# dev-wei/recman

Measured on AMD Instinct MI355X. Metric: examples/sec fwd+bwd, Criteo-shape batch 65536; % HBM and MFMA roofline, higher is better.
Workload: dtype f32; 1 GPU; deepfm (BASELINE configs[1]); batch_per_gpu=65536, batch_all_gpus=65536, sparse_fields=26, rows_per_field=1000001, dense_fields=13, emb_dim=16, indices=uniform, table_row_loads=cached (rm_deepfm_step), row_gradient_stores=cached (as in fit(): the optimizer step gathers them next), optimizer_step=excluded, matrix_arithmetic=f32 MFMA (v_mfma_f32_16x16x4_f32), fp32 accumulate, hipgraph=True, table=single GPU

## Files before the change

### recman_amd/csrc/step.hip

```cpp
#include "mlp_internal.h"
#include "rm_common.h"

namespace {

typedef float f32x4 __attribute__((ext_vector_type(4)));
typedef unsigned u32x4 __attribute__((ext_vector_type(4)));
typedef __amdgpu_buffer_rsrc_t rsrc_t;

constexpr int kWorkers = 7;
constexpr int kSlots = 4;
constexpr int kMaxF = 26;
constexpr int kRing = 3;
constexpr int kSlotB = 1024;
constexpr int kXBufB = kMaxF * kSlotB;
constexpr int kPartH = 0, kPartS = 2048, kPartQ = 3072, kPartSd = 3328, kPartB = 3584;
constexpr int kLDT = 36;
constexpr int kPubDh = 0, kPubDT = 2048, kPubGS = kPubDT + 16 * kLDT * 4, kPubG = kPubGS + 1024, kPubB = kPubG + 256;
constexpr int oX = 0;
constexpr int oDense = oX + kRing * kXBufB;
constexpr int oJunk = oDense + 4 * kSlotB;
constexpr int oZero = oJunk + kSlotB;
constexpr int oPart = oZero + kSlotB;
constexpr int oPub = oPart + 2 * kWorkers * kPartB;
constexpr int kRowB = 28 * 64;
constexpr int oRow = oPub + 2 * kPubB;
constexpr int oHT = oRow + 2 * kRowB;
constexpr int oD1T = oHT + 16 * 32 * 4;
constexpr int oY = oD1T + 16 * 32 * 4;
constexpr int oW1 = oY + 4 * 16 * 4;
constexpr int oPar = oW1 + 32 * 32 * 4;
constexpr int kParB0 = 0, kParB1 = 128, kParWo = 256, kParWd = 384, kParFo = 448;
constexpr int kLdsBytes = oPar + 448 + 28 * 4;
static_assert(kLdsBytes <= 160 * 1024, "LDS map exceeds a CU");

#ifndef RM_STEP_ABL
#define RM_STEP_ABL 0
#endif
#ifdef RM_STEP_STAMP
__device__ unsigned long long rm_step_stamp_buf[256 * 8 * 8];
#define ST_NOW() __builtin_amdgcn_s_memtime()
#define ST_DECL unsigned long long st_acc[8] = {0, 0, 0, 0, 0, 0, 0, 0}, st_t = ST_NOW(), st_t0 = st_t
#define ST_ADD(i) { const unsigned long long st_n = ST_NOW(); st_acc[i] += st_n - st_t; st_t = st_n; }
#define ST_FLUSH(wv) if (lane == 0 && blockIdx.x < 256) { st_acc[7] = ST_NOW() - st_t0; for (int i_ = 0; i_ < 8; ++i_) rm_step_stamp_buf[(blockIdx.x * 8 + (wv)) * 8 + i_] = st_acc[i_]; }
#else
#define ST_DECL
#define ST_ADD(i)
#define ST_FLUSH(wv)
#endif

struct StepArgs {
  const int64_t *idx, *field_off;
  const char *table;
  unsigned row_bytes;
  const float *dense;
  const int64_t *y;
  const float *y_f;
  const float *W0, *b0, *W1, *b1, *w_out, *w0_out, *lin_wd, *lin_w0;
  int F, Dn, H0, H1, act, task, Kp;
  float grad_scale;
  int64_t B;
  float *d_rows, *logit, *pred, *dlogit, *dW0_part, *sg_part, *loss_part;
  int packed, out_row_bytes, out_rows;
  const float *lin_mask;
};

__device__ __forceinline__ float act_slope(int act) {
  return act == RM_ACT_RELU ? 0.f : (act == RM_ACT_LEAKY_RELU ? 0.2f : 1.f);
}
__device__ __forceinline__ float actf(float v, float slope) { return v > 0.f ? v : slope * v; }
__device__ __forceinline__ float actg(float o, float slope) { return o > 0.f ? 1.f : slope; }

__device__ __forceinline__ int slot_field(int w, int j) {
  return j < 3 ? 7 * j + w : (w < 3 ? 21 + w : (w > 3 ? 20 + w : -1));
}

__device__ __forceinline__ f32x4 mfma16(float a, float b, f32x4 c) {
  return __builtin_amdgcn_mfma_f32_16x16x4f32(a, b, c, 0, 0, 0);
}
__device__ __forceinline__ f32x4 mfma16w(float a, float b, f32x4 c) {
  if (RM_STEP_ABL & 16) { c.x += a * b; return c; }
  return __builtin_amdgcn_mfma_f32_16x16x4f32(a, b, c, 0, 0, 0);
}

__device__ __forceinline__ constexpr int swz(int r) { return ((r >> 3) & 1) * 3; }

template <bool NT>
__device__ __forceinline__ void dma16(const char *src, char *lds_dst) {
  __builtin_amdgcn_global_load_lds((const __attribute__((address_space(1))) void *)src,
                                   (__attribute__((address_space(3))) void *)lds_dst, 16, 0, NT ? 2 : 0);
}

template <class T>
__device__ __forceinline__ void entry_load(T &dst, const void *src) {
  static_assert(sizeof(T) == 4, "one dword");
  asm volatile("global_load_dword %0, %1, off" : "=v"(dst) : "v"(src) : "memory");
}
template <int YOUNGER>
__device__ __forceinline__ void entry_wait(float &v) {
  asm volatile("s_waitcnt vmcnt(%1)" : "+v"(v) : "n"(YOUNGER) : "memory");
}

typedef float f32x2 __attribute__((ext_vector_type(2)));
template <int OFF, class T>
__device__ __forceinline__ void lds_load(T &dst, unsigned addr) {
  static_assert(sizeof(T) == 4 || sizeof(T) == 16, "b32 or b128");
  if (sizeof(T) == 4) asm volatile("ds_read_b32 %0, %1 offset:%2" : "=v"(dst) : "v"(addr), "n"(OFF) : "memory");
  else asm volatile("ds_read_b128 %0, %1 offset:%2" : "=v"(dst) : "v"(addr), "n"(OFF) : "memory");
}
__device__ __forceinline__ void lds_load_pair(f32x2 &dst, unsigned addr) {
  asm volatile("ds_read2st64_b32 %0, %1 offset1:1" : "=v"(dst) : "v"(addr) : "memory");
}
struct SlotRegs {
  f32x2 col[2];
  f32x4 e4;
};
#define RM_SLOT_REGS(r) "+v"((r).col[0]), "+v"((r).col[1]), "+v"((r).e4)
template <bool PACKED>
__device__ __forceinline__ void slot_wait0(f32x4 (&dhB)[2], float (&dT)[2][4], f32x4 &gS, float &g, unsigned (&rid)[4],
                                           unsigned (&rp0)[4], SlotRegs &r) {
  if (PACKED)
    asm volatile("s_waitcnt lgkmcnt(9)"
                 : "+v"(dhB[0]), "+v"(dhB[1]), "+v"(dT[0][0]), "+v"(dT[0][1]), "+v"(dT[0][2]), "+v"(dT[0][3]),
                   "+v"(dT[1][0]), "+v"(dT[1][1]), "+v"(dT[1][2]), "+v"(dT[1][3]), "+v"(gS), "+v"(g), "+v"(rid[0]),
                   "+v"(rid[1]), "+v"(rid[2]), "+v"(rid[3]), "+v"(rp0[0]), "+v"(rp0[1]), "+v"(rp0[2]), "+v"(rp0[3]),
                   RM_SLOT_REGS(r)::"memory");
  else
    asm volatile("s_waitcnt lgkmcnt(9)"
                 : "+v"(dhB[0]), "+v"(dhB[1]), "+v"(dT[0][0]), "+v"(dT[0][1]), "+v"(dT[0][2]), "+v"(dT[0][3]),
                   "+v"(dT[1][0]), "+v"(dT[1][1]), "+v"(dT[1][2]), "+v"(dT[1][3]), "+v"(gS), "+v"(g), "+v"(rid[0]),
                   "+v"(rid[1]), "+v"(rid[2]), "+v"(rid[3]), RM_SLOT_REGS(r)::"memory");
}
__device__ __forceinline__ void slot_wait(int j, SlotRegs &r) {
  if (j == 1) asm volatile("s_waitcnt lgkmcnt(6)" : RM_SLOT_REGS(r)::"memory");
  else if (j == 2) asm volatile("s_waitcnt lgkmcnt(3)" : RM_SLOT_REGS(r)::"memory");
  else asm volatile("s_waitcnt lgkmcnt(0)" : RM_SLOT_REGS(r)::"memory");
}
static_assert(kSlots == 4, "slot_wait's counts");

__device__ __forceinline__ void wait_vm(int younger) {
#define RM_WV(N) case N: asm volatile("s_waitcnt vmcnt(" #N ")" ::: "memory"); break;
  switch (younger) {
    RM_WV(24) RM_WV(23) RM_WV(22) RM_WV(21) RM_WV(20) RM_WV(19) RM_WV(18) RM_WV(17) RM_WV(16) RM_WV(15) RM_WV(14) RM_WV(13) RM_WV(12) RM_WV(11) RM_WV(10) RM_WV(9) RM_WV(8) RM_WV(7) RM_WV(6)
    RM_WV(5) RM_WV(4) RM_WV(3) RM_WV(2) RM_WV(1)
    default: asm volatile("s_waitcnt vmcnt(0)" ::: "memory"); break;
  }
#undef RM_WV
}

__device__ __forceinline__ void tile_barrier() {
  asm volatile("s_waitcnt lgkmcnt(0)" ::: "memory");
  __builtin_amdgcn_s_barrier();
  asm volatile("" ::: "memory");
}

__device__ __forceinline__ float sum_q(float v) {
  {
    float a = v, c = v;
    asm("s_nop 1\n\tv_permlane16_swap_b32 %0, %1" : "+v"(a), "+v"(c));
    v = a + c;
  }
  {
    float a = v, c = v;
    asm("s_nop 1\n\tv_permlane32_swap_b32 %0, %1" : "+v"(a), "+v"(c));
    v = a + c;
  }
  return v;
}
__device__ __forceinline__ float sum_n(float v) {
#pragma unroll
  for (int o = 1; o < 16; o <<= 1) v += __shfl_xor(v, o, 64);
  return v;
}

template <bool NT, bool NT_OUT, bool PACKED>
__device__ __forceinline__ void step_worker(const StepArgs &a, char *smem, const int w, const int lane, const int T) {
  const int n = lane & 15, q = lane >> 4;
  const int F = a.F, H0 = a.H0, K = 16 * F + a.Dn;
  int fld[kSlots];
  bool sv[kSlots], sx[kSlots];
  float w0f[kSlots][2][4];
  float w0x[kSlots][2][4];
  f32x4 dw[kSlots][2];
#pragma unroll
  for (int j = 0; j < kSlots; ++j) {
    const int f = slot_field(w, j);
    sv[j] = f >= 0 && (f < F || (f == F && a.Dn > 0));
    sx[j] = f >= 0 && f < F;
    fld[j] = sv[j] ? f : 0;
    const int kb = 16 * fld[j];
#pragma unroll
    for (int uh = 0; uh < 2; ++uh) {
#pragma unroll
      for (int e = 0; e < 4; ++e) {
        const int kf = kb + 4 * q + e, uf = 16 * uh + n;
        const bool okf = sv[j] && kf < K && uf < H0;
        const float vf = a.W0[okf ? (int64_t)kf * H0 + uf : 0];
        w0f[j][uh][e] = okf ? vf : 0.f;
        const int kx = kb + n, ux = 16 * uh + 4 * q + e;
        const bool okx = sx[j] && kx < K && ux < H0;
        const float vx = a.W0[okx ? (int64_t)kx * H0 + ux : 0];
        w0x[j][uh][e] = okx ? vx : 0.f;
      }
      dw[j][uh] = f32x4{0.f, 0.f, 0.f, 0.f};
    }
  }
  const int64_t tstride = gridDim.x;
  const int lo_slice = n * 64 + 16 * (q ^ swz(n));
  int lo_col[2];
#pragma unroll
  for (int h = 0; h < 2; ++h) lo_col[h] = (8 * h + q) * 64 + 16 * ((n >> 2) ^ swz(8 * h + q)) + 4 * (n & 3);
  static_assert(swz(0) == swz(4) && swz(3) == swz(7) && swz(8) == swz(12) && swz(11) == swz(15), "a pair of column reads shares its swizzle");
  const unsigned lds0 = (unsigned)(uintptr_t)(__attribute__((address_space(3))) char *)smem;
  const int lo_row = n * F * 64 + 16 * q;
  auto slot_base = [&](int j, int tile) {
    const int ring = oX + ((tile + 6) % 3) * kXBufB + fld[j] * kSlotB, dn = oDense + (tile & 3) * kSlotB;
    return __builtin_amdgcn_readfirstlane(sx[j] ? ring : (sv[j] ? dn : oZero));
  };
  *reinterpret_cast<f32x4 *>(smem + oZero + lane * 16) = f32x4{0.f, 0.f, 0.f, 0.f};
  const int piece = 16 * ((lane & 3) ^ swz(lane >> 2));
  const int side_off = 64 + 4 * (lane & 1);
  float sdv[kSlots];
#pragma unroll
  for (int j = 0; j < kSlots; ++j) sdv[j] = 0.f;
  unsigned rp[4][kSlots];
  float lmask[kSlots];
#pragma unroll
  for (int j = 0; j < kSlots; ++j) {
    rp[0][j] = rp[1][j] = rp[2][j] = rp[3][j] = 0;
    lmask[j] = (PACKED && a.lin_mask != nullptr && sx[j]) ? a.lin_mask[fld[j]] : 1.f;
  }
  constexpr int kSP = PACKED ? 2 : 1;
  constexpr int kYoungerE = 7 + 4 * kSP, kYounger = 8 + 6 * kSP;
  static_assert(kYounger <= 24, "wait_vm's range");
  asm volatile("" ::"s"(a.row_bytes) : "memory");
  ST_DECL;
  ST_ADD(0);

  for (int s = -2; s <= T + 1; ++s) {
    const bool hasB = s - 2 >= 0 && s - 2 < T;
    const bool hasD = s + 1 >= 0 && s + 1 < T;
    float side_sum = 0.f;
    {
      const int tb = s - 2, td = s + 1;
      char *xd = smem + oX + ((td + 3) % 3) * kXBufB;
      f32x4 dhB[2], gS;
      float dT[2][4], g;
      SlotRegs sr[kSlots];
      unsigned rid[kSlots];
      {
        const unsigned pub = lds0 + oPub + (tb & 1) * kPubB;
        lds_load<kPubDh>(dhB[0], pub + lane * 16);
        lds_load<kPubDh + 1024>(dhB[1], pub + lane * 16);
        const unsigned pt = pub + (q * kLDT + n) * 4;
#pragma unroll
        for (int uh = 0; uh < 2; ++uh) {
          lds_load<kPubDT + (0 * 4 * kLDT) * 4>(dT[uh][0], pt + 64 * uh);
          lds_load<kPubDT + (1 * 4 * kLDT) * 4>(dT[uh][1], pt + 64 * uh);
          lds_load<kPubDT + (2 * 4 * kLDT) * 4>(dT[uh][2], pt + 64 * uh);
          lds_load<kPubDT + (3 * 4 * kLDT) * 4>(dT[uh][3], pt + 64 * uh);
        }
        lds_load<kPubGS>(gS, pub + lane * 16);
        lds_load<kPubG>(g, pub + lane * 4);
      }
      if (PACKED) {
#pragma unroll
        for (int j = 0; j < kSlots; ++j) {
          rp[3][j] = rp[2][j];
          rp[2][j] = rp[1][j];
          rp[1][j] = rp[0][j];
        }
      }
// ... 84 lines not shown
      }
    }
    ST_ADD(6);
    if (s >= 0 && s < T) {
      wait_vm(kYounger);
      ST_ADD(3);
      f32x4 acc0 = f32x4{0.f, 0.f, 0.f, 0.f}, acc1 = acc0, S = acc0, Q = acc0;
      f32x4 x4[kSlots];
#pragma unroll
      for (int j = 0; j < kSlots; ++j) {
        x4[j] = *reinterpret_cast<const f32x4 *>(smem + slot_base(j, s) + lo_slice);
      }
#pragma unroll
      for (int j = 0; j < kSlots; ++j) {
#pragma unroll
        for (int ks = 0; ks < 4; ++ks) {
          acc0 = mfma16w(w0f[j][0][ks], x4[j][ks], acc0);
          acc1 = mfma16w(w0f[j][1][ks], x4[j][ks], acc1);
        }
        const float m = sx[j] ? 1.f : 0.f;
        S += m * x4[j];
        Q += m * (x4[j] * x4[j]);
      }
      char *part = smem + oPart + ((s & 1) * kWorkers + w) * kPartB;
      *reinterpret_cast<f32x4 *>(part + kPartH + lane * 16) = acc0;
      *reinterpret_cast<f32x4 *>(part + kPartH + (64 + lane) * 16) = acc1;
      *reinterpret_cast<f32x4 *>(part + kPartS + lane * 16) = S;
      *reinterpret_cast<float *>(part + kPartQ + lane * 4) = (Q.x + Q.y) + (Q.z + Q.w);
      *reinterpret_cast<float *>(part + kPartSd + lane * 4) = side_sum;
    }
    ST_ADD(4);
    tile_barrier();
    ST_ADD(5);
  }
  asm volatile("s_waitcnt vmcnt(0)" ::: "memory");
#pragma unroll
  for (int j = 0; j < kSlots; ++j)
    if (sv[j]) {
#pragma unroll
      for (int uh = 0; uh < 2; ++uh)
#pragma unroll
        for (int i = 0; i < 4; ++i)
          a.dW0_part[((int64_t)blockIdx.x * a.Kp + 16 * fld[j] + 4 * q + i) * 32 + 16 * uh + n] = dw[j][uh][i];
    }
  ST_ADD(0);
  ST_FLUSH(w);
}

__device__ __forceinline__ void step_head(const StepArgs &a, char *smem, const int lane, const int T) {
  const int n = lane & 15, q = lane >> 4;
  const int F = a.F, Dn = a.Dn, H0 = a.H0, H1 = a.H1;
  const float act = act_slope(a.act);
  const int64_t B = a.B, tstride = gridDim.x;
  {
    float *w1s = reinterpret_cast<float *>(smem + oW1);
#pragma unroll
    for (int i = 0; i < 16; ++i) {
      const int e = lane + 64 * i, u = e >> 5, v = e & 31;
      const bool ok = u < H0 && v < H1;
      const float f = a.W1[ok ? u * H1 + v : 0];
      w1s[u * 32 + 4 * ((v >> 2) ^ (u & 7)) + (v & 3)] = ok ? f : 0.f;
    }
    float *par = reinterpret_cast<float *>(smem + oPar);
    if (lane < 32) {
      const float f0 = a.b0[lane < H0 ? lane : 0], f1 = a.b1[lane < H1 ? lane : 0], f2 = a.w_out[lane < H1 ? lane : 0];
      par[kParB0 / 4 + lane] = lane < H0 ? f0 : 0.f;
      par[kParB1 / 4 + lane] = lane < H1 ? f1 : 0.f;
      par[kParWo / 4 + lane] = lane < H1 ? f2 : 0.f;
      const float f3 = a.lin_wd[lane < Dn ? lane : 0];
      if (lane < 16) par[kParWd / 4 + lane] = lane < Dn ? f3 : 0.f;
      if (lane < 28) reinterpret_cast<unsigned *>(par)[kParFo / 4 + lane] = (unsigned)a.field_off[lane < F ? lane : F - 1];
    }
  }
  const float *w1s = reinterpret_cast<const float *>(smem + oW1);
  const char *par = smem + oPar;
  const float w0o = a.w0_out[0], lw0 = a.lin_w0[0];

  f32x4 dW1[2][2];
  float db0[2][4], db1[2][4], dwo[2][4], dxd[4], sg = 0.f, loss_acc = 0.f;
#pragma unroll
  for (int x = 0; x < 2; ++x)
#pragma unroll
    for (int i = 0; i < 4; ++i) {
      dW1[x][0][i] = dW1[x][1][i] = 0.f;
      db0[x][i] = db1[x][i] = dwo[x][i] = 0.f;
    }
#pragma unroll
  for (int i = 0; i < 4; ++i) dxd[i] = 0.f;

  auto ex_of = [&](int t) {
    const int64_t b = ((int64_t)blockIdx.x + t * tstride) * 16 + n;
    return b < B ? b : B - 1;
  };
  unsigned idr[7];
  float dnr[4];
  unsigned yr = 0;
#pragma unroll
  for (int j = 0; j < 7; ++j) idr[j] = 0;
#pragma unroll
  for (int i = 0; i < 4; ++i) dnr[i] = 0.f;
  auto load_ids = [&](int t) {
    const unsigned *p = reinterpret_cast<const unsigned *>(a.idx + ex_of(t) * F);
#pragma unroll
    for (int j = 0; j < 7; ++j) entry_load(idr[j], p + 2 * (q + 4 * j < F ? q + 4 * j : F - 1));
  };
  asm volatile("" ::"v"(w0o), "v"(lw0) : "memory");
  load_ids(0);
  ST_DECL;
  ST_ADD(0);

  for (int s = -2; s <= T + 1; ++s) {
    const bool epi = s - 1 >= 0 && s - 1 < T;
    float o_z = 0.f, o_p = 0.f, o_g = 0.f;
    if (epi) {
      const int t = s - 1;
      const int64_t bex = ((int64_t)blockIdx.x + t * tstride) * 16 + n;
      const bool valid = bex < B;
      f32x4 pre[2], S = f32x4{0.f, 0.f, 0.f, 0.f};
      pre[0] = pre[1] = S;
      float ss = 0.f, y1 = 0.f, ls = 0.f;
#pragma unroll
      for (int w = 0; w < kWorkers; ++w) {
        const char *part = smem + oPart + ((t & 1) * kWorkers + w) * kPartB;
        pre[0] += *reinterpret_cast<const f32x4 *>(part + kPartH + lane * 16);
        pre[1] += *reinterpret_cast<const f32x4 *>(part + kPartH + (64 + lane) * 16);
        S += *reinterpret_cast<const f32x4 *>(part + kPartS + lane * 16);
        ss += *reinterpret_cast<const float *>(part + kPartQ + lane * 4);
        const float2 sd = *reinterpret_cast<const float2 *>(part + kPartSd + 16 * n);
        y1 += sd.x;
        ls += sd.y;
        if (w == 3) __builtin_amdgcn_sched_barrier(0);
      }
      const f32x4 dn4 = Dn > 0 ? *reinterpret_cast<const f32x4 *>(smem + oDense + (t & 3) * kSlotB + n * 64 + 16 * (q ^ swz(n)))
                               : f32x4{0.f, 0.f, 0.f, 0.f};
      const f32x4 wdv = *reinterpret_cast<const f32x4 *>(par + kParWd + 16 * q);
      const float fmq = sum_q(S.x * S.x + S.y * S.y + S.z * S.z + S.w * S.w - ss);
      const float lind = sum_q(dn4.x * wdv.x + dn4.y * wdv.y + dn4.z * wdv.z + dn4.w * wdv.w);
      const float fm = y1 + 0.5f * fmq;
      const float lin = ls + lind + lw0;
      const float ty = *reinterpret_cast<const float *>(smem + oY + ((t & 3) * 16 + n) * 4);
      ST_ADD(1);
      float h0[2][4], h1[2][4];
#pragma unroll
      for (int h = 0; h < 2; ++h) {
        const f32x4 b0v = *reinterpret_cast<const f32x4 *>(par + kParB0 + (16 * h + 4 * q) * 4);
#pragma unroll
        for (int i = 0; i < 4; ++i) h0[h][i] = actf(pre[h][i] + b0v[i], act);
        *reinterpret_cast<f32x4 *>(smem + oHT + (n * 32 + 16 * h + 4 * q) * 4) =
            f32x4{h0[h][0], h0[h][1], h0[h][2], h0[h][3]};
      }
      f32x4 acc[2];
      acc[0] = acc[1] = f32x4{0.f, 0.f, 0.f, 0.f};
#pragma unroll
      for (int uh = 0; uh < 2; ++uh)
#pragma unroll
        for (int i = 0; i < 4; ++i) {
          const int u = 16 * uh + 4 * q + i;
          const float a0 = w1s[u * 32 + 4 * ((n >> 2) ^ (u & 7)) + (n & 3)];
          const float a1 = w1s[u * 32 + 4 * ((4 + (n >> 2)) ^ (u & 7)) + (n & 3)];
          acc[0] = mfma16(a0, h0[uh][i], acc[0]);
          acc[1] = mfma16(a1, h0[uh][i], acc[1]);
        }
      float dnn = 0.f;
      f32x4 wov[2];
#pragma unroll
      for (int h = 0; h < 2; ++h) {
        const f32x4 b1v = *reinterpret_cast<const f32x4 *>(par + kParB1 + (16 * h + 4 * q) * 4);
        wov[h] = *reinterpret_cast<const f32x4 *>(par + kParWo + (16 * h + 4 * q) * 4);
#pragma unroll
        for (int i = 0; i < 4; ++i) {
          h1[h][i] = actf(acc[h][i] + b1v[i], act);
          dnn += h1[h][i] * wov[h][i];
        }
      }
      dnn = sum_q(dnn) + w0o;
      float z = 0.f;
      z += lin;
      z += fm;
      z += dnn;
      float p, dz;
      const float lt = rm_loss_point(z, ty, a.task, &p, &dz);
      float gb = dz * (1.0f / (float)B);
      gb *= a.grad_scale;
      gb = valid ? gb : 0.f;
      o_z = z;
      o_p = p;
      o_g = gb;
      if (valid && q == 0) loss_acc += lt;
      ST_ADD(2);
      float dh1[2][4], dh0[2][4];
#pragma unroll
      for (int h = 0; h < 2; ++h) {
#pragma unroll
        for (int i = 0; i < 4; ++i) dh1[h][i] = gb * wov[h][i] * actg(h1[h][i], act);
        *reinterpret_cast<f32x4 *>(smem + oD1T + (n * 32 + 16 * h + 4 * q) * 4) =
            f32x4{dh1[h][0], dh1[h][1], dh1[h][2], dh1[h][3]};
      }
      acc[0] = acc[1] = f32x4{0.f, 0.f, 0.f, 0.f};
#pragma unroll
      for (int vh = 0; vh < 2; ++vh) {
        const f32x4 c0 = *reinterpret_cast<const f32x4 *>(w1s + n * 32 + 4 * ((4 * vh + q) ^ (n & 7)));
        const f32x4 c1 = *reinterpret_cast<const f32x4 *>(w1s + (16 + n) * 32 + 4 * ((4 * vh + q) ^ (n & 7)));
#pragma unroll
        for (int i = 0; i < 4; ++i) {
          acc[0] = mfma16(c0[i], dh1[vh][i], acc[0]);
          acc[1] = mfma16(c1[i], dh1[vh][i], acc[1]);
        }
      }
      char *pub = smem + oPub + (t & 1) * kPubB;
#pragma unroll
      for (int h = 0; h < 2; ++h) {
#pragma unroll
        for (int i = 0; i < 4; ++i) dh0[h][i] = acc[h][i] * actg(h0[h][i], act);
        const f32x4 d4 = f32x4{dh0[h][0], dh0[h][1], dh0[h][2], dh0[h][3]};
        *reinterpret_cast<f32x4 *>(pub + kPubDh + (h * 64 + lane) * 16) = d4;
        *reinterpret_cast<f32x4 *>(pub + kPubDT + (n * kLDT + 16 * h + 4 * q) * 4) = d4;
      }
      *reinterpret_cast<f32x4 *>(pub + kPubGS + lane * 16) = f32x4{gb * S.x, gb * S.y, gb * S.z, gb * S.w};
      *reinterpret_cast<float *>(pub + kPubG + lane * 4) = gb;
      ST_ADD(3);
#pragma unroll
      for (int es = 0; es < 4; ++es) {
        float av[2], bv[2];
#pragma unroll
        for (int h = 0; h < 2; ++h) {
          av[h] = *reinterpret_cast<const float *>(smem + oHT + ((4 * es + q) * 32 + 16 * h + n) * 4);
          bv[h] = *reinterpret_cast<const float *>(smem + oD1T + ((4 * es + q) * 32 + 16 * h + n) * 4);
        }
#pragma unroll
        for (int uh = 0; uh < 2; ++uh)
#pragma unroll
          for (int vh = 0; vh < 2; ++vh) dW1[uh][vh] = mfma16(av[uh], bv[vh], dW1[uh][vh]);
      }
#pragma unroll
      for (int h = 0; h < 2; ++h)
#pragma unroll
        for (int i = 0; i < 4; ++i) {
          db0[h][i] += dh0[h][i];
          db1[h][i] += dh1[h][i];
          dwo[h][i] += gb * h1[h][i];
        }
      sg += q == 0 ? gb : 0.f;
      dxd[0] += gb * dn4.x;
      dxd[1] += gb * dn4.y;
      dxd[2] += gb * dn4.z;
      dxd[3] += gb * dn4.w;
    }
    ST_ADD(4);
    {
      const int64_t ex0 = epi ? ((int64_t)blockIdx.x + (s - 1) * tstride) * 16 : 0;
      const int64_t left = B - ex0;
      const int nb = epi ? 4 * (left < 16 ? (int)left : 16) : 0;
      const int off = q == 0 ? 4 * n : 0x7ffffff0;
      __builtin_amdgcn_raw_buffer_store_b32(__float_as_uint(o_z), __builtin_amdgcn_make_buffer_rsrc(a.logit + ex0, 0, nb, 0x00020000), off, 0, 0);
      __builtin_amdgcn_raw_buffer_store_b32(__float_as_uint(o_p), __builtin_amdgcn_make_buffer_rsrc(a.pred + ex0, 0, nb, 0x00020000), off, 0, 0);
      __builtin_amdgcn_raw_buffer_store_b32(__float_as_uint(o_g), __builtin_amdgcn_make_buffer_rsrc(a.dlogit + ex0, 0, nb, 0x00020000), off, 0, 0);
    }
    asm volatile("s_waitcnt vmcnt(10)" : "+v"(dnr[0]), "+v"(dnr[1]), "+v"(dnr[2]), "+v"(dnr[3]), "+v"(yr)::"memory");
    if (s + 1 >= 0 && s + 1 < T) {
      const int t = s + 1;
      if (Dn > 0)
        *reinterpret_cast<f32x4 *>(smem + oDense + (t & 3) * kSlotB + n * 64 + 16 * (q ^ swz(n))) =
            f32x4{4 * q + 0 < Dn ? dnr[0] : 0.f, 4 * q + 1 < Dn ? dnr[1] : 0.f, 4 * q + 2 < Dn ? dnr[2] : 0.f,
                  4 * q + 3 < Dn ? dnr[3] : 0.f};
      if (q == 0)
        *reinterpret_cast<float *>(smem + oY + ((t & 3) * 16 + n) * 4) = a.y ? (float)(int)yr : __uint_as_float(yr);
    }
    asm volatile("s_waitcnt vmcnt(3)"
                 : "+v"(idr[0]), "+v"(idr[1]), "+v"(idr[2]), "+v"(idr[3]), "+v"(idr[4]), "+v"(idr[5]), "+v"(idr[6])::"memory");
    if (s + 2 < T) {
      unsigned *rowid = reinterpret_cast<unsigned *>(smem + oRow + ((s + 2) & 1) * kRowB);
#pragma unroll
      for (int j = 0; j < 7; ++j)
        rowid[(q + 4 * j) * 16 + n] = idr[j] + *reinterpret_cast<const unsigned *>(par + kParFo + (q + 4 * j) * 4);
    }
    __builtin_amdgcn_sched_barrier(0);
    {
      const int64_t b = ex_of(s + 2);
      const float *dp = Dn > 0 ? a.dense + b * Dn : a.w_out;
#pragma unroll
      for (int i = 0; i < 4; ++i) entry_load(dnr[i], dp + (4 * q + i < Dn ? 4 * q + i : 0));
      const unsigned *yp = a.y ? reinterpret_cast<const unsigned *>(a.y + b) : reinterpret_cast<const unsigned *>(a.y_f + b);
      entry_load(yr, yp);
    }
    load_ids(s + 3);
    ST_ADD(6);
    tile_barrier();
    ST_ADD(5);
  }

  asm volatile("s_waitcnt vmcnt(0)" ::: "memory");
  float *sgp = a.sg_part + (int64_t)blockIdx.x * kRmSgStride;
#pragma unroll
  for (int uh = 0; uh < 2; ++uh)
#pragma unroll
    for (int vh = 0; vh < 2; ++vh)
#pragma unroll
      for (int i = 0; i < 4; ++i) sgp[(16 * uh + 4 * q + i) * 32 + 16 * vh + n] = dW1[uh][vh][i];
#pragma unroll
  for (int h = 0; h < 2; ++h)
#pragma unroll
    for (int i = 0; i < 4; ++i) {
      const float s0 = sum_n(db0[h][i]), s1 = sum_n(db1[h][i]), s2 = sum_n(dwo[h][i]);
      if (n == 0) {
        const int u = 16 * h + 4 * q + i;
        sgp[2 * 1024 + u] = s0;
        sgp[2 * 1024 + 32 + u] = s1;
        sgp[2 * 1024 + 64 + u] = s2;
      }
    }
#pragma unroll
  for (int i = 0; i < 4; ++i) {
    const float sx = sum_n(dxd[i]);
    if (n == 0) sgp[kRmSgDense + 4 * q + i] = sx;
  }
  const float sgt = rm_wave_sum(sg), lst = rm_wave_sum(loss_acc);
  if (lane == 0) {
    sgp[2 * 1024 + 64 + 32] = sgt;
    a.loss_part[blockIdx.x] = lst;
  }
  ST_ADD(0);
  ST_FLUSH(7);
}

template <bool NT, bool NT_OUT, bool PACKED>
__global__ __launch_bounds__(512) void deepfm_step_kernel(StepArgs a) {
  extern __shared__ __attribute__((aligned(16))) char smem[];
  const int lane = threadIdx.x & 63;
  const int wave = __builtin_amdgcn_readfirstlane(threadIdx.x >> 6);
  const int64_t ntiles = (a.B + 15) / 16;
  const int T = (int)((ntiles - blockIdx.x + gridDim.x - 1) / gridDim.x);
#ifndef RM_STEP_PRIO
#define RM_STEP_PRIO 1
#endif
  if (wave < kWorkers) {
    if (RM_STEP_PRIO == 1 && wave >= 4) __builtin_amdgcn_s_setprio(1);
    step_worker<NT, NT_OUT, PACKED>(a, smem, wave, lane, T);
  } else {
    if (RM_STEP_PRIO) __builtin_amdgcn_s_setprio(2);
    step_head(a, smem, lane, T);
  }
}

constexpr int kCuLdsBytes = 160 * 1024;
static_assert(kLdsBytes <= kCuLdsBytes, "the fill must cover the step's allocation");

__global__ __launch_bounds__(512) void lds_fill_kernel(unsigned pattern) {
  extern __shared__ __attribute__((aligned(16))) char smem[];
  volatile unsigned *p = reinterpret_cast<volatile unsigned *>(smem);
  for (int pass = 0; pass < 2; ++pass) {
    for (int i = threadIdx.x; i < kCuLdsBytes / 4; i += 512) p[i] = pattern;
    __syncthreads();
  }
}

__global__ __launch_bounds__(64) void lds_probe_kernel(unsigned pattern, unsigned *mismatches) {
  extern __shared__ __attribute__((aligned(16))) char smem[];
  const volatile unsigned *p = reinterpret_cast<const volatile unsigned *>(smem);
  unsigned n = 0;
  for (int i = threadIdx.x; i < kCuLdsBytes / 4; i += 64) n += p[i] != pattern;
  for (int off = 32; off > 0; off >>= 1) n += __shfl_xor(n, off, 64);
  if (threadIdx.x == 0) mismatches[blockIdx.x] = n;
}

}

static int lds_aid_cus(const void *kernel, const char *who, int *cus) {
  int dev = 0, lds = 0;
  RM_REQUIRE(hipGetDevice(&dev) == hipSuccess &&
                 hipDeviceGetAttribute(cus, hipDeviceAttributeMultiprocessorCount, dev) == hipSuccess && *cus > 0 &&
                 hipDeviceGetAttribute(&lds, hipDeviceAttributeMaxSharedMemoryPerBlock, dev) == hipSuccess,
             "%s: no device", who);
// ... 100 lines not shown
```

Before: 658.7 million examples/s.

## Software-pipeline LDS reads in step head and use scalar-base global loads

The head wave now issues all partial-sum LDS reads before accumulating, and hoists bias, dense, weight and HT/D1T operand reads so they interleave with the MFMA chains, pinned in place with sched_barrier. Global loads for ids, dense and labels switch to scalar-base plus 32-bit lane offset addressing with incrementally advanced tile offsets, replacing per-lane 64-bit address math. Field offsets move from LDS into registers. The aim is to cut LDS latency stalls and VALU address overhead on the serial head wave, at the cost of higher register pressure.

New measurement: 663.2 million examples/s (median of 6 runs). About the same (+0.7%).

```diff
diff --git a/recman_amd/csrc/step.hip b/recman_amd/csrc/step.hip
--- a/recman_amd/csrc/step.hip
+++ b/recman_amd/csrc/step.hip
@@ -29,8 +29,8 @@
 constexpr int oY = oD1T + 16 * 32 * 4;
 constexpr int oW1 = oY + 4 * 16 * 4;
 constexpr int oPar = oW1 + 32 * 32 * 4;
-constexpr int kParB0 = 0, kParB1 = 128, kParWo = 256, kParWd = 384, kParFo = 448;
-constexpr int kLdsBytes = oPar + 448 + 28 * 4;
+constexpr int kParB0 = 0, kParB1 = 128, kParWo = 256, kParWd = 384;
+constexpr int kLdsBytes = oPar + 448;
 static_assert(kLdsBytes <= 160 * 1024, "LDS map exceeds a CU");
 
 #ifndef RM_STEP_ABL
@@ -94,6 +94,11 @@
 __device__ __forceinline__ void entry_load(T &dst, const void *src) {
   static_assert(sizeof(T) == 4, "one dword");
   asm volatile("global_load_dword %0, %1, off" : "=v"(dst) : "v"(src) : "memory");
+}
+template <class T>
+__device__ __forceinline__ void entry_load_at(T &dst, const void *base, unsigned off) {
+  static_assert(sizeof(T) == 4, "one dword");
+  asm volatile("global_load_dword %0, %1, %2" : "=v"(dst) : "v"(off), "s"(base) : "memory");
 }
 template <int YOUNGER>
 __device__ __forceinline__ void entry_wait(float &v) {
@@ -153,6 +158,16 @@
   asm volatile("" ::: "memory");
 }
 
+__device__ __forceinline__ void read_fence() {
+  asm volatile("" ::: "memory");
+  __builtin_amdgcn_sched_barrier(0);
+}
+
+__device__ __forceinline__ void pin_order() {
+  asm volatile("" ::: "memory");
+  __builtin_amdgcn_sched_barrier(0x476);
+}
+
 __device__ __forceinline__ float sum_q(float v) {
   {
     float a = v, c = v;
@@ -424,7 +439,6 @@
       par[kParWo / 4 + lane] = lane < H1 ? f2 : 0.f;
       const float f3 = a.lin_wd[lane < Dn ? lane : 0];
       if (lane < 16) par[kParWd / 4 + lane] = lane < Dn ? f3 : 0.f;
-      if (lane < 28) reinterpret_cast<unsigned *>(par)[kParFo / 4 + lane] = (unsigned)a.field_off[lane < F ? lane : F - 1];
     }
   }
   const float *w1s = reinterpret_cast<const float *>(smem + oW1);
@@ -443,9 +457,19 @@
 #pragma unroll
   for (int i = 0; i < 4; ++i) dxd[i] = 0.f;
 
-  auto ex_of = [&](int t) {
-    const int64_t b = ((int64_t)blockIdx.x + t * tstride) * 16 + n;
-    return b < B ? b : B - 1;
+  const int64_t tstep = 16 * tstride;
+  const int64_t stepD = tstep * Dn, stepF = tstep * F, lastD = (B - 1) * Dn, lastF = (B - 1) * F;
+  const unsigned rowD = 4u * Dn, rowF = 8u * F;
+  const int ysh = a.y ? 3 : 2;
+  const char *ybase = a.y ? reinterpret_cast<const char *>(a.y) : reinterpret_cast<const char *>(a.y_f);
+  unsigned coD[4], coF[7];
+#pragma unroll
+  for (int i = 0; i < 4; ++i) coD[i] = 4u * (4 * q + i < Dn ? 4 * q + i : 0);
+#pragma unroll
+  for (int j = 0; j < 7; ++j) coF[j] = 8u * (q + 4 * j < F ? q + 4 * j : F - 1);
+  auto lane_clamp = [&](int64_t left) {
+    const int last = left > 0 ? (left < 16 ? (int)left : 16) - 1 : 0;
+    return (unsigned)(n < last ? n : last);
   };
   unsigned idr[7];
   float dnr[4];
@@ -454,13 +478,21 @@
   for (int j = 0; j < 7; ++j) idr[j] = 0;
 #pragma unroll
   for (int i = 0; i < 4; ++i) dnr[i] = 0.f;
-  auto load_ids = [&](int t) {
-    const unsigned *p = reinterpret_cast<const unsigned *>(a.idx + ex_of(t) * F);
-#pragma unroll
-    for (int j = 0; j < 7; ++j) entry_load(idr[j], p + 2 * (q + 4 * j < F ? q + 4 * j : F - 1));
+  auto load_ids = [&](int64_t tile0, int64_t off) {
+    const int64_t left = B - tile0;
+    const int64_t *base = a.idx + (left > 0 ? off : lastF);
+    const unsigned nc = lane_clamp(left);
+#pragma unroll
+    for (int j = 0; j < 7; ++j) entry_load_at(idr[j], base, __umul24(nc, rowF) + coF[j]);
   };
-  asm volatile("" ::"v"(w0o), "v"(lw0) : "memory");
-  load_ids(0);
+  unsigned fo[7];
+#pragma unroll
+  for (int j = 0; j < 7; ++j) fo[j] = (unsigned)a.field_off[q + 4 * j < F ? q + 4 * j : F - 1];
+  asm volatile("" ::"v"(w0o), "v"(lw0), "v"(fo[0]), "v"(fo[1]), "v"(fo[2]), "v"(fo[3]), "v"(fo[4]), "v"(fo[5]), "v"(fo[6])
+               : "memory");
+  int64_t tile2 = (int64_t)blockIdx.x * 16, offD = tile2 * Dn;
+  load_ids(tile2, tile2 * F);
+  int64_t tile3 = tile2 + tstep, offF = tile3 * F;
   ST_DECL;
   ST_ADD(0);
 
@@ -474,57 +506,96 @@
       f32x4 pre[2], S = f32x4{0.f, 0.f, 0.f, 0.f};
       pre[0] = pre[1] = S;
       float ss = 0.f, y1 = 0.f, ls = 0.f;
+      f32x4 b0v[2], ph[kWorkers][2], pS[kWorkers];
+      float pq[kWorkers];
+      float2 psd[kWorkers];
+#pragma unroll
+      for (int h = 0; h < 2; ++h) b0v[h] = *reinterpret_cast<const f32x4 *>(par + kParB0 + (16 * h + 4 * q) * 4);
 #pragma unroll
       for (int w = 0; w < kWorkers; ++w) {
         const char *part = smem + oPart + ((t & 1) * kWorkers + w) * kPartB;
-        pre[0] += *reinterpret_cast<const f32x4 *>(part + kPartH + lane * 16);
-        pre[1] += *reinterpret_cast<const f32x4 *>(part + kPartH + (64 + lane) * 16);
-        S += *reinterpret_cast<const f32x4 *>(part + kPartS + lane * 16);
-        ss += *reinterpret_cast<const float *>(part + kPartQ + lane * 4);
-        const float2 sd = *reinterpret_cast<const float2 *>(part + kPartSd + 16 * n);
-        y1 += sd.x;
-        ls += sd.y;
-        if (w == 3) __builtin_amdgcn_sched_barrier(0);
-      }
-      const f32x4 dn4 = Dn > 0 ? *reinterpret_cast<const f32x4 *>(smem + oDense + (t & 3) * kSlotB + n * 64 + 16 * (q ^ swz(n)))
-                               : f32x4{0.f, 0.f, 0.f, 0.f};
-      const f32x4 wdv = *reinterpret_cast<const f32x4 *>(par + kParWd + 16 * q);
+        ph[w][0] = *reinterpret_cast<const f32x4 *>(part + kPartH + lane * 16);
+        ph[w][1] = *reinterpret_cast<const f32x4 *>(part + kPartH + (64 + lane) * 16);
+        pS[w] = *reinterpret_cast<const f32x4 *>(part + kPartS + lane * 16);
+        pq[w] = *reinterpret_cast<const float *>(part + kPartQ + lane * 4);
+        psd[w] = *reinterpret_cast<const float2 *>(part + kPartSd + 16 * n);
+      }
+      read_fence();
+#pragma unroll
+      for (int w = 0; w < kWorkers; ++w) {
+        pre[0] += ph[w][0];
+        pre[1] += ph[w][1];
+        S += pS[w];
+        ss += pq[w];
+        y1 += psd[w].x;
+        ls += psd[w].y;
+      }
       const float fmq = sum_q(S.x * S.x + S.y * S.y + S.z * S.z + S.w * S.w - ss);
-      const float lind = sum_q(dn4.x * wdv.x + dn4.y * wdv.y + dn4.z * wdv.z + dn4.w * wdv.w);
       const float fm = y1 + 0.5f * fmq;
-      const float lin = ls + lind + lw0;
-      const float ty = *reinterpret_cast<const float *>(smem + oY + ((t & 3) * 16 + n) * 4);
       ST_ADD(1);
       float h0[2][4], h1[2][4];
 #pragma unroll
       for (int h = 0; h < 2; ++h) {
-        const f32x4 b0v = *reinterpret_cast<const f32x4 *>(par + kParB0 + (16 * h + 4 * q) * 4);
-#pragma unroll
-        for (int i = 0; i < 4; ++i) h0[h][i] = actf(pre[h][i] + b0v[i], act);
+#pragma unroll
+        for (int i = 0; i < 4; ++i) h0[h][i] = actf(pre[h][i] + b0v[h][i], act);
         *reinterpret_cast<f32x4 *>(smem + oHT + (n * 32 + 16 * h + 4 * q) * 4) =
             f32x4{h0[h][0], h0[h][1], h0[h][2], h0[h][3]};
       }
+      float a0[2][4], a1[2][4];
+#pragma unroll
+      for (int i = 0; i < 4; ++i) {
+        const int u = 4 * q + i;
+        const float *p0 = w1s + u * 32 + 4 * ((n >> 2) ^ (u & 7)) + (n & 3);
+        const float *p1 = w1s + u * 32 + 4 * ((4 + (n >> 2)) ^ (u & 7)) + (n & 3);
+        a0[0][i] = p0[0];
+        a0[1][i] = p0[16 * 32];
+        a1[0][i] = p1[0];
+        a1[1][i] = p1[16 * 32];
+      }
+      f32x4 dn4 = f32x4{0.f, 0.f, 0.f, 0.f}, wdv, b1v[2], wov[2], c0[2], c1[2];
+      float ty;
+      pin_order();
       f32x4 acc[2];
       acc[0] = acc[1] = f32x4{0.f, 0.f, 0.f, 0.f};
 #pragma unroll
-      for (int uh = 0; uh < 2; ++uh)
+      for (int uh = 0; uh < 2; ++uh) {
 #pragma unroll
         for (int i = 0; i < 4; ++i) {
-          const int u = 16 * uh + 4 * q + i;
-          const float a0 = w1s[u * 32 + 4 * ((n >> 2) ^ (u & 7)) + (n & 3)];
-          const float a1 = w1s[u * 32 + 4 * ((4 + (n >> 2)) ^ (u & 7)) + (n & 3)];
-          acc[0] = mfma16(a0, h0[uh][i], acc[0]);
-          acc[1] = mfma16(a1, h0[uh][i], acc[1]);
-        }
+          acc[0] = mfma16(a0[uh][i], h0[uh][i], acc[0]);
+          pin_order();
+          acc[1] = mfma16(a1[uh][i], h0[uh][i], acc[1]);
+          pin_order();
+          if (uh > 0) continue;
+          if (i == 0) {
+            if (Dn > 0) dn4 = *reinterpret_cast<const f32x4 *>(smem + oDense + (t & 3) * kSlotB + n * 64 + 16 * (q ^ swz(n)));
+            wdv = *reinterpret_cast<const f32x4 *>(par + kParWd + 16 * q);
+            ty = *reinterpret_cast<const float *>(smem + oY + ((t & 3) * 16 + n) * 4);
+          }
+          if (i == 1) {
+#pragma unroll
+            for (int h = 0; h < 2; ++h) {
+              b1v[h] = *reinterpret_cast<const f32x4 *>(par + kParB1 + (16 * h + 4 * q) * 4);
+              wov[h] = *reinterpret_cast<const f32x4 *>(par + kParWo + (16 * h + 4 * q) * 4);
+            }
+          }
+          if (i == 2) {
+#pragma unroll
+            for (int vh = 0; vh < 2; ++vh) {
+              c0[vh] = *reinterpret_cast<const f32x4 *>(w1s + n * 32 + 4 * ((4 * vh + q) ^ (n & 7)));
+              c1[vh] = *reinterpret_cast<const f32x4 *>(w1s + (16 + n) * 32 + 4 * ((4 * vh + q) ^ (n & 7)));
+            }
+          }
+          pin_order();
+        }
+      }
+      const float lind = sum_q(dn4.x * wdv.x + dn4.y * wdv.y + dn4.z * wdv.z + dn4.w * wdv.w);
+      const float lin = ls + lind + lw0;
       float dnn = 0.f;
-      f32x4 wov[2];
 #pragma unroll
       for (int h = 0; h < 2; ++h) {
-        const f32x4 b1v = *reinterpret_cast<const f32x4 *>(par + kParB1 + (16 * h + 4 * q) * 4);
-        wov[h] = *reinterpret_cast<const f32x4 *>(par + kParWo + (16 * h + 4 * q) * 4);
 #pragma unroll
         for (int i = 0; i < 4; ++i) {
-          h1[h][i] = actf(acc[h][i] + b1v[i], act);
+          h1[h][i] = actf(acc[h][i] + b1v[h][i], act);
           dnn += h1[h][i] * wov[h][i];
         }
       }
@@ -552,14 +623,23 @@
             f32x4{dh1[h][0], dh1[h][1], dh1[h][2], dh1[h][3]};
       }
       acc[0] = acc[1] = f32x4{0.f, 0.f, 0.f, 0.f};
+      float av[4][2], bv[4][2];
 #pragma unroll
       for (int vh = 0; vh < 2; ++vh) {
-        const f32x4 c0 = *reinterpret_cast<const f32x4 *>(w1s + n * 32 + 4 * ((4 * vh + q) ^ (n & 7)));
-        const f32x4 c1 = *reinterpret_cast<const f32x4 *>(w1s + (16 + n) * 32 + 4 * ((4 * vh + q) ^ (n & 7)));
 #pragma unroll
         for (int i = 0; i < 4; ++i) {
-          acc[0] = mfma16(c0[i], dh1[vh][i], acc[0]);
-          acc[1] = mfma16(c1[i], dh1[vh][i], acc[1]);
+          acc[0] = mfma16(c0[vh][i], dh1[vh][i], acc[0]);
+          pin_order();
+          acc[1] = mfma16(c1[vh][i], dh1[vh][i], acc[1]);
+          pin_order();
+          if (vh > 0) continue;
+#pragma unroll
+          for (int h = 0; h < 2; ++h) {
+            const float *ht = reinterpret_cast<const float *>(smem + oHT) + (4 * i + q) * 32 + 16 * h + n;
+            av[i][h] = ht[0];
+            bv[i][h] = ht[(oD1T - oHT) / 4];
+          }
+          pin_order();
         }
       }
       char *pub = smem + oPub + (t & 1) * kPubB;
@@ -573,20 +653,14 @@
       }
       *reinterpret_cast<f32x4 *>(pub + kPubGS + lane * 16) = f32x4{gb * S.x, gb * S.y, gb * S.z, gb * S.w};
       *reinterpret_cast<float *>(pub + kPubG + lane * 4) = gb;
+      __builtin_amdgcn_sched_barrier(0);
       ST_ADD(3);
 #pragma unroll
-      for (int es = 0; es < 4; ++es) {
-        float av[2], bv[2];
-#pragma unroll
-        for (int h = 0; h < 2; ++h) {
-          av[h] = *reinterpret_cast<const float *>(smem + oHT + ((4 * es + q) * 32 + 16 * h + n) * 4);
-          bv[h] = *reinterpret_cast<const float *>(smem + oD1T + ((4 * es + q) * 32 + 16 * h + n) * 4);
-        }
+      for (int es = 0; es < 4; ++es)
 #pragma unroll
         for (int uh = 0; uh < 2; ++uh)
 #pragma unroll
-          for (int vh = 0; vh < 2; ++vh) dW1[uh][vh] = mfma16(av[uh], bv[vh], dW1[uh][vh]);
-      }
+          for (int vh = 0; vh < 2; ++vh) dW1[uh][vh] = mfma16(av[es][uh], bv[es][vh], dW1[uh][vh]);
 #pragma unroll
       for (int h = 0; h < 2; ++h)
 #pragma unroll
@@ -627,18 +701,22 @@
       unsigned *rowid = reinterpret_cast<unsigned *>(smem + oRow + ((s + 2) & 1) * kRowB);
 #pragma unroll
       for (int j = 0; j < 7; ++j)
-        rowid[(q + 4 * j) * 16 + n] = idr[j] + *reinterpret_cast<const unsigned *>(par + kParFo + (q + 4 * j) * 4);
+        rowid[(q + 4 * j) * 16 + n] = idr[j] + fo[j];
     }
     __builtin_amdgcn_sched_barrier(0);
     {
-      const int64_t b = ex_of(s + 2);
-      const float *dp = Dn > 0 ? a.dense + b * Dn : a.w_out;
-#pragma unroll
-      for (int i = 0; i < 4; ++i) entry_load(dnr[i], dp + (4 * q + i < Dn ? 4 * q + i : 0));
-      const unsigned *yp = a.y ? reinterpret_cast<const unsigned *>(a.y + b) : reinterpret_cast<const unsigned *>(a.y_f + b);
-      entry_load(yr, yp);
-    }
-    load_ids(s + 3);
+      const int64_t left = B - tile2;
+      const float *dbase = Dn > 0 ? a.dense + (left > 0 ? offD : lastD) : a.w_out;
+      const unsigned nc = lane_clamp(left);
+#pragma unroll
+      for (int i = 0; i < 4; ++i) entry_load_at(dnr[i], dbase, __umul24(nc, rowD) + coD[i]);
+      entry_load_at(yr, ybase + ((left > 0 ? tile2 : B - 1) << ysh), nc << ysh);
+    }
+    load_ids(tile3, offF);
+    tile2 = tile3;
+    tile3 += tstep;
+    offD += stepD;
+    offF += stepF;
     ST_ADD(6);
     tile_barrier();
     ST_ADD(5);
@@ -693,6 +771,7 @@
     step_worker<NT, NT_OUT, PACKED>(a, smem, wave, lane, T);
   } else {
     if (RM_STEP_PRIO) __builtin_amdgcn_s_setprio(2);
+    asm volatile("" : "+s"(a.grad_scale));
     step_head(a, smem, lane, T);
   }
 }
```

## Peel pipeline prologue, vectorize W0 transpose loads, overlap setup loads

Applied to the files above, without the earlier changes.

Vectorizes the transposed W0 register load into 16-byte loads when W0 is aligned and H0 is a multiple of 4. In the producer wave it issues the W1/parameter global loads before the LDS writes, and peels the first pipeline iteration into explicit setup followed by a barrier. The loop then starts one stage later. The aim is to shorten kernel prologue latency by overlapping the index, W1 and parameter loads and by cutting scalar load instructions. It also extends the optional timing stamps with per-segment classes. The risk is very small because the prologue is a small part of a long persistent loop.

After: 670.2 million examples/s before, 684.5 million examples/s after, median of 6. +2.1%, better.

```diff
diff --git a/recman_amd/csrc/step.hip b/recman_amd/csrc/step.hip
--- a/recman_amd/csrc/step.hip
+++ b/recman_amd/csrc/step.hip
@@ -37,14 +37,35 @@
 #define RM_STEP_ABL 0
 #endif
 #ifdef RM_STEP_STAMP
-__device__ unsigned long long rm_step_stamp_buf[256 * 8 * 8];
+constexpr int kStampC = 9, kStampW = 8 + 2 * kStampC;
+__device__ unsigned long long rm_step_stamp_buf[256 * 8 * kStampW];
 #define ST_NOW() __builtin_amdgcn_s_memtime()
-#define ST_DECL unsigned long long st_acc[8] = {0, 0, 0, 0, 0, 0, 0, 0}, st_t = ST_NOW(), st_t0 = st_t
-#define ST_ADD(i) { const unsigned long long st_n = ST_NOW(); st_acc[i] += st_n - st_t; st_t = st_n; }
-#define ST_FLUSH(wv) if (lane == 0 && blockIdx.x < 256) { st_acc[7] = ST_NOW() - st_t0; for (int i_ = 0; i_ < 8; ++i_) rm_step_stamp_buf[(blockIdx.x * 8 + (wv)) * 8 + i_] = st_acc[i_]; }
+#define ST_DECL                                                                                                   \
+  unsigned long long st_acc[8] = {0, 0, 0, 0, 0, 0, 0, 0}, st_cls[kStampC] = {0, 0, 0, 0, 0, 0, 0, 0, 0},            \
+                     st_clb[kStampC] = {0, 0, 0, 0, 0, 0, 0, 0, 0}, st_t = ST_NOW(), st_t0 = st_t, st_seg = st_t, st_d = 0
+#define ST_ADD(i) { const unsigned long long st_n = ST_NOW(); st_d = st_n - st_t; st_acc[i] += st_d; st_t = st_n; }
+#define ST_CLS(c, bar)                                                                                            \
+  {                                                                                                               \
+    const int st_c = (c);                                                                                         \
+    const unsigned long long st_e = st_t - st_seg;                                                                \
+    st_seg = st_t;                                                                                                \
+    _Pragma("unroll") for (int i_ = 0; i_ < kStampC; ++i_) {                                                      \
+      st_cls[i_] += i_ == st_c ? st_e : 0ull;                                                                     \
+      st_clb[i_] += ((bar) && i_ == st_c) ? st_d : 0ull;                                                          \
+    }                                                                                                             \
+  }
+#define ST_SEG_CLASS(s, T) ((s) < 2 ? (s) + 3 : ((s) < (T) ? 5 : (s) - (T) + 6))
+#define ST_FLUSH(wv)                                                                                              \
+  if (lane == 0 && blockIdx.x < 256) {                                                                            \
+    st_acc[7] = ST_NOW() - st_t0;                                                                                 \
+    unsigned long long *st_o = rm_step_stamp_buf + (blockIdx.x * 8 + (wv)) * kStampW;                             \
+    for (int i_ = 0; i_ < 8; ++i_) st_o[i_] = st_acc[i_];                                                         \
+    for (int i_ = 0; i_ < kStampC; ++i_) { st_o[8 + i_] = st_cls[i_]; st_o[8 + kStampC + i_] = st_clb[i_]; }      \
+  }
 #else
 #define ST_DECL
 #define ST_ADD(i)
+#define ST_CLS(c, bar)
 #define ST_FLUSH(wv)
 #endif
 
@@ -176,6 +197,8 @@
 __device__ __forceinline__ void step_worker(const StepArgs &a, char *smem, const int w, const int lane, const int T) {
   const int n = lane & 15, q = lane >> 4;
   const int F = a.F, H0 = a.H0, K = 16 * F + a.Dn;
+  ST_DECL;
+  const bool w0_x4 = (((uintptr_t)a.W0 & 15) | (unsigned)(H0 & 3)) == 0;
   int fld[kSlots];
   bool sv[kSlots], sx[kSlots];
   float w0f[kSlots][2][4];
@@ -196,13 +219,41 @@
         const bool okf = sv[j] && kf < K && uf < H0;
         const float vf = a.W0[okf ? (int64_t)kf * H0 + uf : 0];
         w0f[j][uh][e] = okf ? vf : 0.f;
-        const int kx = kb + n, ux = 16 * uh + 4 * q + e;
-        const bool okx = sx[j] && kx < K && ux < H0;
-        const float vx = a.W0[okx ? (int64_t)kx * H0 + ux : 0];
-        w0x[j][uh][e] = okx ? vx : 0.f;
       }
       dw[j][uh] = f32x4{0.f, 0.f, 0.f, 0.f};
     }
+  }
+  if (w0_x4) {
+    f32x4 vx[kSlots][2];
+    bool okx[kSlots][2];
+#pragma unroll
+    for (int j = 0; j < kSlots; ++j)
+#pragma unroll
+      for (int uh = 0; uh < 2; ++uh) {
+        const int kx = 16 * fld[j] + n, ux = 16 * uh + 4 * q;
+        okx[j][uh] = sx[j] && kx < K && ux < H0;
+        vx[j][uh] = *reinterpret_cast<const f32x4 *>(a.W0 + (okx[j][uh] ? (int64_t)kx * H0 + ux : 0));
+      }
+    asm volatile("" : "+v"(vx[0][0]), "+v"(vx[0][1]), "+v"(vx[1][0]), "+v"(vx[1][1]), "+v"(vx[2][0]), "+v"(vx[2][1]),
+                      "+v"(vx[3][0]), "+v"(vx[3][1])::"memory");
+#pragma unroll
+    for (int j = 0; j < kSlots; ++j)
+#pragma unroll
+      for (int uh = 0; uh < 2; ++uh)
+#pragma unroll
+        for (int e = 0; e < 4; ++e) w0x[j][uh][e] = okx[j][uh] ? vx[j][uh][e] : 0.f;
+  } else {
+#pragma unroll
+    for (int j = 0; j < kSlots; ++j)
+#pragma unroll
+      for (int uh = 0; uh < 2; ++uh)
+#pragma unroll
+        for (int e = 0; e < 4; ++e) {
+          const int kx = 16 * fld[j] + n, ux = 16 * uh + 4 * q + e;
+          const bool okx = sx[j] && kx < K && ux < H0;
+          const float vx = a.W0[okx ? (int64_t)kx * H0 + ux : 0];
+          w0x[j][uh][e] = okx ? vx : 0.f;
+        }
   }
   const int64_t tstride = gridDim.x;
   const int lo_slice = n * 64 + 16 * (q ^ swz(n));
@@ -233,10 +284,12 @@
   constexpr int kYoungerE = 7 + 4 * kSP, kYounger = 8 + 6 * kSP;
   static_assert(kYounger <= 24, "wait_vm's range");
   asm volatile("" ::"s"(a.row_bytes) : "memory");
-  ST_DECL;
   ST_ADD(0);
-
-  for (int s = -2; s <= T + 1; ++s) {
+  tile_barrier();
+  ST_ADD(5);
+  ST_CLS(0, true);
+
+  for (int s = -1; s <= T + 1; ++s) {
     const bool hasB = s - 2 >= 0 && s - 2 < T;
     const bool hasD = s + 1 >= 0 && s + 1 < T;
     float side_sum = 0.f;
@@ -387,6 +440,7 @@
     ST_ADD(4);
     tile_barrier();
     ST_ADD(5);
+    ST_CLS(ST_SEG_CLASS(s, T), true);
   }
   asm volatile("s_waitcnt vmcnt(0)" ::: "memory");
 #pragma unroll
@@ -399,6 +453,7 @@
           a.dW0_part[((int64_t)blockIdx.x * a.Kp + 16 * fld[j] + 4 * q + i) * 32 + 16 * uh + n] = dw[j][uh][i];
     }
   ST_ADD(0);
+  ST_CLS(8, false);
   ST_FLUSH(w);
 }
 
@@ -407,42 +462,7 @@
   const int F = a.F, Dn = a.Dn, H0 = a.H0, H1 = a.H1;
   const float act = act_slope(a.act);
   const int64_t B = a.B, tstride = gridDim.x;
-  {
-    float *w1s = reinterpret_cast<float *>(smem + oW1);
-#pragma unroll
-    for (int i = 0; i < 16; ++i) {
-      const int e = lane + 64 * i, u = e >> 5, v = e & 31;
-      const bool ok = u < H0 && v < H1;
-      const float f = a.W1[ok ? u * H1 + v : 0];
-      w1s[u * 32 + 4 * ((v >> 2) ^ (u & 7)) + (v & 3)] = ok ? f : 0.f;
-    }
-    float *par = reinterpret_cast<float *>(smem + oPar);
-    if (lane < 32) {
-      const float f0 = a.b0[lane < H0 ? lane : 0], f1 = a.b1[lane < H1 ? lane : 0], f2 = a.w_out[lane < H1 ? lane : 0];
-      par[kParB0 / 4 + lane] = lane < H0 ? f0 : 0.f;
-      par[kParB1 / 4 + lane] = lane < H1 ? f1 : 0.f;
-      par[kParWo / 4 + lane] = lane < H1 ? f2 : 0.f;
-      const float f3 = a.lin_wd[lane < Dn ? lane : 0];
-      if (lane < 16) par[kParWd / 4 + lane] = lane < Dn ? f3 : 0.f;
-      if (lane < 28) reinterpret_cast<unsigned *>(par)[kParFo / 4 + lane] = (unsigned)a.field_off[lane < F ? lane : F - 1];
-    }
-  }
-  const float *w1s = reinterpret_cast<const float *>(smem + oW1);
-  const char *par = smem + oPar;
-  const float w0o = a.w0_out[0], lw0 = a.lin_w0[0];
-
-  f32x4 dW1[2][2];
-  float db0[2][4], db1[2][4], dwo[2][4], dxd[4], sg = 0.f, loss_acc = 0.f;
-#pragma unroll
-  for (int x = 0; x < 2; ++x)
-#pragma unroll
-    for (int i = 0; i < 4; ++i) {
-      dW1[x][0][i] = dW1[x][1][i] = 0.f;
-      db0[x][i] = db1[x][i] = dwo[x][i] = 0.f;
-    }
-#pragma unroll
-  for (int i = 0; i < 4; ++i) dxd[i] = 0.f;
-
+  ST_DECL;
   auto ex_of = [&](int t) {
     const int64_t b = ((int64_t)blockIdx.x + t * tstride) * 16 + n;
     return b < B ? b : B - 1;
@@ -459,12 +479,76 @@
 #pragma unroll
     for (int j = 0; j < 7; ++j) entry_load(idr[j], p + 2 * (q + 4 * j < F ? q + 4 * j : F - 1));
   };
-  asm volatile("" ::"v"(w0o), "v"(lw0) : "memory");
   load_ids(0);
-  ST_DECL;
+  float w0o, lw0;
+  {
+    float w1v[16];
+#pragma unroll
+    for (int i = 0; i < 16; ++i) {
+      const int e = lane + 64 * i, u = e >> 5, v = e & 31;
+      w1v[i] = a.W1[(u < H0 && v < H1) ? u * H1 + v : 0];
+    }
+    const int l32 = lane & 31;
+    const float f0 = a.b0[l32 < H0 ? l32 : 0], f1 = a.b1[l32 < H1 ? l32 : 0], f2 = a.w_out[l32 < H1 ? l32 : 0];
+    const float f3 = a.lin_wd[l32 < Dn ? l32 : 0];
+    const unsigned fo = (unsigned)a.field_off[l32 < F ? l32 : F - 1];
+    w0o = a.w0_out[0];
+    lw0 = a.lin_w0[0];
+    asm volatile("" ::"v"(f3), "v"(fo), "v"(w0o), "v"(lw0) : "memory");
+    float *w1s = reinterpret_cast<float *>(smem + oW1);
+#pragma unroll
+    for (int i = 0; i < 16; ++i) {
+      const int e = lane + 64 * i, u = e >> 5, v = e & 31;
+      w1s[u * 32 + 4 * ((v >> 2) ^ (u & 7)) + (v & 3)] = (u < H0 && v < H1) ? w1v[i] : 0.f;
+    }
+    float *par = reinterpret_cast<float *>(smem + oPar);
+    if (lane < 32) {
+      par[kParB0 / 4 + lane] = lane < H0 ? f0 : 0.f;
+      par[kParB1 / 4 + lane] = lane < H1 ? f1 : 0.f;
+      par[kParWo / 4 + lane] = lane < H1 ? f2 : 0.f;
+      if (lane < 16) par[kParWd / 4 + lane] = lane < Dn ? f3 : 0.f;
+      if (lane < 28) reinterpret_cast<unsigned *>(par)[kParFo / 4 + lane] = fo;
+    }
+  }
+  const float *w1s = reinterpret_cast<const float *>(smem + oW1);
+  const char *par = smem + oPar;
+
+  f32x4 dW1[2][2];
+  float db0[2][4], db1[2][4], dwo[2][4], dxd[4], sg = 0.f, loss_acc = 0.f;
+#pragma unroll
+  for (int x = 0; x < 2; ++x)
+#pragma unroll
+    for (int i = 0; i < 4; ++i) {
+      dW1[x][0][i] = dW1[x][1][i] = 0.f;
+      db0[x][i] = db1[x][i] = dwo[x][i] = 0.f;
+    }
+#pragma unroll
+  for (int i = 0; i < 4; ++i) dxd[i] = 0.f;
+
+  asm volatile("s_waitcnt vmcnt(0)"
+               : "+v"(idr[0]), "+v"(idr[1]), "+v"(idr[2]), "+v"(idr[3]), "+v"(idr[4]), "+v"(idr[5]), "+v"(idr[6])::"memory");
+  {
+    unsigned *rowid = reinterpret_cast<unsigned *>(smem + oRow);
+#pragma unroll
+    for (int j = 0; j < 7; ++j)
+      rowid[(q + 4 * j) * 16 + n] = idr[j] + *reinterpret_cast<const unsigned *>(par + kParFo + (q + 4 * j) * 4);
+  }
+  __builtin_amdgcn_sched_barrier(0);
+  {
+    const int64_t b = ex_of(0);
+    const float *dp = Dn > 0 ? a.dense + b * Dn : a.w_out;
+#pragma unroll
+    for (int i = 0; i < 4; ++i) entry_load(dnr[i], dp + (4 * q + i < Dn ? 4 * q + i : 0));
+    const unsigned *yp = a.y ? reinterpret_cast<const unsigned *>(a.y + b) : reinterpret_cast<const unsigned *>(a.y_f + b);
+    entry_load(yr, yp);
+  }
+  load_ids(1);
   ST_ADD(0);
-
-  for (int s = -2; s <= T + 1; ++s) {
+  tile_barrier();
+  ST_ADD(5);
+  ST_CLS(0, true);
+
+  for (int s = -1; s <= T + 1; ++s) {
     const bool epi = s - 1 >= 0 && s - 1 < T;
     float o_z = 0.f, o_p = 0.f, o_g = 0.f;
     if (epi) {
@@ -642,39 +726,46 @@
     ST_ADD(6);
     tile_barrier();
     ST_ADD(5);
+    ST_CLS(ST_SEG_CLASS(s, T), true);
   }
 
   asm volatile("s_waitcnt vmcnt(0)" ::: "memory");
-  float *sgp = a.sg_part + (int64_t)blockIdx.x * kRmSgStride;
-#pragma unroll
-  for (int uh = 0; uh < 2; ++uh)
-#pragma unroll
-    for (int vh = 0; vh < 2; ++vh)
-#pragma unroll
-      for (int i = 0; i < 4; ++i) sgp[(16 * uh + 4 * q + i) * 32 + 16 * vh + n] = dW1[uh][vh][i];
-#pragma unroll
-  for (int h = 0; h < 2; ++h)
+  int el = lane;
+  asm volatile("" : "+v"(el));
+  {
+    const int n = el & 15, q = el >> 4;
+    float *sgp = a.sg_part + (int64_t)blockIdx.x * kRmSgStride;
+#pragma unroll
+    for (int uh = 0; uh < 2; ++uh)
+#pragma unroll
+      for (int vh = 0; vh < 2; ++vh)
+#pragma unroll
+        for (int i = 0; i < 4; ++i) sgp[(16 * uh + 4 * q + i) * 32 + 16 * vh + n] = dW1[uh][vh][i];
+#pragma unroll
+    for (int h = 0; h < 2; ++h)
+#pragma unroll
+      for (int i = 0; i < 4; ++i) {
+        const float s0 = sum_n(db0[h][i]), s1 = sum_n(db1[h][i]), s2 = sum_n(dwo[h][i]);
+        if (n == 0) {
+          const int u = 16 * h + 4 * q + i;
+          sgp[2 * 1024 + u] = s0;
+          sgp[2 * 1024 + 32 + u] = s1;
+          sgp[2 * 1024 + 64 + u] = s2;
+        }
+      }
 #pragma unroll
     for (int i = 0; i < 4; ++i) {
-      const float s0 = sum_n(db0[h][i]), s1 = sum_n(db1[h][i]), s2 = sum_n(dwo[h][i]);
-      if (n == 0) {
-        const int u = 16 * h + 4 * q + i;
-        sgp[2 * 1024 + u] = s0;
-        sgp[2 * 1024 + 32 + u] = s1;
-        sgp[2 * 1024 + 64 + u] = s2;
-      }
-    }
-#pragma unroll
-  for (int i = 0; i < 4; ++i) {
-    const float sx = sum_n(dxd[i]);
-    if (n == 0) sgp[kRmSgDense + 4 * q + i] = sx;
-  }
-  const float sgt = rm_wave_sum(sg), lst = rm_wave_sum(loss_acc);
-  if (lane == 0) {
-    sgp[2 * 1024 + 64 + 32] = sgt;
-    a.loss_part[blockIdx.x] = lst;
+      const float sx = sum_n(dxd[i]);
+      if (n == 0) sgp[kRmSgDense + 4 * q + i] = sx;
+    }
+    const float sgt = rm_wave_sum(sg), lst = rm_wave_sum(loss_acc);
+    if (lane == 0) {
+      sgp[2 * 1024 + 64 + 32] = sgt;
+      a.loss_part[blockIdx.x] = lst;
+    }
   }
   ST_ADD(0);
+  ST_CLS(8, false);
   ST_FLUSH(7);
 }
 
```
